# toverainc/willow-inference-server

Hardware: AMD Instinct MI355X
Metric: realtime_multiple (audio_ms / infer_ms), Whisper large-v2 beam=5, 3.84 s clip (higher is better)
Workload: dtype f16; 1 GPU; whisper-large beam=5 clip=3sec (3840 ms) batch=1/GPU, PCM resident in HBM -> ids on host; parallelism=1 independent replicas (utterance sharding, no data-path collective)

## Files before the change

### include/wis_hip.h

```cpp
#ifndef WIS_HIP_H
#define WIS_HIP_H

#include <stddef.h>
#include <stdint.h>

#ifdef __cplusplus
extern "C" {
#endif

#define WIS_ABI_VERSION 1

#define WIS_OK             0
#define WIS_E_ARG         -1
#define WIS_E_FORMAT      -2
#define WIS_E_NOMEM       -3
#define WIS_E_CHECKSUM    -4
#define WIS_E_HIP         -5
#define WIS_E_STATE       -6
#define WIS_E_UNSUPPORTED -7

#define WIS_SAMPLE_RATE 16000
#define WIS_N_FFT       400
#define WIS_HOP         160
#define WIS_N_MELS      80
// ... 136 lines not shown
int wis_align_last_timing(wis_model_t* m, float* ms);
int wis_op_dtw(int device, const float* x, int N, int M, int32_t* text_idx, int32_t* time_idx, int32_t* len);
int wis_op_align_matrix(int device, const float* q, const void* kx_f16, int T_tokens, int n_heads_sel, int T, int frames, int width, float* out);
int wis_debug_tree_logits(wis_model_t* m, const float* input, int input_kind, const int32_t* prompt, int P, int beam,
                          const int32_t* tok, const int32_t* org, int n_steps, float* logits);

int wis_debug_search(wis_model_t* m, const float* logits, int n_steps, int B, const wis_gen_opts_t* opts,
                     int32_t* out_ids, int32_t* out_len, float* out_score, int32_t* out_finish_step, int32_t* out_parent);
int wis_debug_search_n(wis_model_t* m, const float* logits, int n_steps, int B, const wis_gen_opts_t* opts, const uint64_t* seeds, const uint32_t* noise,
                       int32_t* out_ids, int32_t* out_len, float* out_score, int32_t* out_finish_step, int32_t* out_parent);

int wis_debug_handoff(wis_model_t* m, int raise_flag, int* retries, int* spin_disabled);
int wis_debug_graph_count(wis_model_t* m, int* count);
int wis_debug_sa_long(wis_model_t* m, int form);

typedef struct {
  float logmel_ms, encoder_ms, crosskv_ms, prefill_ms, decode_ms, total_ms;
  int32_t decode_steps;
  int32_t decode_steps_needed;
} wis_timing_t;
int wis_last_timing(const wis_model_t* m, wis_timing_t* t);

int wis_debug_phase_cycles(wis_model_t* m, int B, int beam, int pos, uint64_t* out);

int wis_debug_timeline(wis_model_t* m, int B, int beam, int pos, int use_graph, uint64_t* out, int n_out);
int wis_debug_sampling_cycles(wis_model_t* m, uint64_t* out);

int wis_bench_weight_stream(wis_model_t* m, int M, int passes, float* total_ms, int* launches_per_pass,
                            double* bytes_per_pass);

int wis_dev_alloc(int device, size_t bytes, void** out);
int wis_dev_free(int device, void* p);
int wis_dev_h2d(int device, void* dst, const void* src, size_t bytes);
int wis_dev_d2h(int device, void* dst, const void* src, size_t bytes);
int wis_dev_sync(int device);
int wis_dev_copy_peer(int dst_device, void* dst, int src_device, const void* src, size_t bytes);

int wis_op_gemm(int device, const void* A_f16, int lda, const void* W_f16, const float* bias,
                const float* residual, void* C, int M, int N, int K, int flags);
int wis_op_layernorm(int device, const float* x, const float* gamma, const float* beta,
                     void* y_f16, int M, int d);
int wis_op_enc_attention(int device, const void* qk_f16, const void* vt_f16, void* out_f16,
                         int B, int T, int Tpad, int H);
int wis_op_enc_attention_ex(int device, const void* qk_f16, const void* vt_f16, void* out_f16,
                            int B, int T, int Tpad, int H, int form);
int wis_op_gemv(int device, const void* x, const float* gamma, const float* beta,
// ... 91 lines not shown
```

### willow-inference-server_amd/csrc/dec_kernels.hip

```cpp
#include <string.h>
#include "common.hpp"
#include "kernels.hpp"

namespace wis {

__global__ void pack_gemv_kernel(const f16* __restrict__ W, f16* __restrict__ Wp, int N, int Npad, int K, int n_scale, float scale, int rows) {
  const int ksteps = K / 32;
  const size_t total = (size_t)Npad * ksteps * 4;
  for (size_t idx = (size_t)blockIdx.x * blockDim.x + threadIdx.x; idx < total; idx += (size_t)gridDim.x * blockDim.x) {
    const int row = (int)(idx % rows);
    size_t t = idx / rows;
    const int kq = (int)(t & 3); t >>= 2;
    const int ks = (int)(t % ksteps), nt = (int)(t / ksteps);
    const int n = rows * nt + row, k = 32 * ks + 8 * kq;
    f16x8 v;
    if (n < N) {
      v = *reinterpret_cast<const f16x8*>(W + (size_t)n * K + k);
      if (n < n_scale) {
#pragma unroll
        for (int j = 0; j < 8; ++j) v[j] = (f16)((float)v[j] * scale);
      }
    } else {
#pragma unroll
      for (int j = 0; j < 8; ++j) v[j] = (f16)0.f;
// ... 495 lines not shown
      if ((lane >> 4) == 0 && m < M && rows * tile < p.N) *reinterpret_cast<float2*>(p.stat_out + ((size_t)m * (p.N >> 4) + tile) * 2) = make_float2(t1, t2);
    }
  }
  stamp(pf, 6);
  if (tid == 0) tl_end(p.prof);
#undef WIS_ROW_OF
}
#define WIS_GV_LEAD(q) (q).x, (q).x2, (q).Wp, (q).M, (q).N, (q).K, (q).xsplit
#define WIS_GV_LEAD_DECL(s) const void* s##x, const void* s##x2, const f16* s##Wp, int s##M, int s##N, int s##K, int s##xsplit
#define WIS_GV_LEAD_APPLY(q, s) (q).x = s##x; (q).x2 = s##x2; (q).Wp = s##Wp; (q).M = s##M; (q).N = s##N; (q).K = s##K; (q).xsplit = s##xsplit
template <int MB, int MODE, int SC, int RM, bool W8, int NT = 1, int NC = 16>
__global__ __launch_bounds__(256) void gemv_kernel(WIS_GV_LEAD_DECL(l_), int KC, GemvP p) {
  extern __shared__ __attribute__((aligned(16))) char smem[];
  WIS_GV_LEAD_APPLY(p, l_);
  gemv_body<MB, MODE, SC, RM, W8, NT, NC>(p, KC, blockIdx.x, smem);
}
template <int SCA, int SCB>
__global__ __launch_bounds__(256) void gemv_dual_kernel(int nA, int M, const void* ax, const f16* aWp, const void* bx, const void* bx2, const f16* bWp, int bxsplit,
                                                        GemvP pa, GemvP pb) {
  extern __shared__ __attribute__((aligned(16))) char smem[];
  if ((int)blockIdx.x < nA) { pa.x = ax; pa.x2 = nullptr; pa.Wp = aWp; pa.M = M; pa.K = SCA * 128; gemv_body<1, 2, SCA, 1, false>(pa, SCA * 128, blockIdx.x, smem); }
  else { pb.x = bx; pb.x2 = bx2; pb.Wp = bWp; pb.M = M; pb.K = SCB * 128; pb.xsplit = bxsplit; gemv_body<1, 2, SCB, 1, false>(pb, SCB * 128, (int)blockIdx.x - nA, smem); }
}
int launch_gemv_dual(hipStream_t st, const GemvP& pa, const GemvP& pb) {
  if (pa.M != pb.M || pa.M < 1 || pa.M > 16 || pa.x2 || pa.wscale || pb.wscale || (pa.flags & (GV_LN | GV_QKV)) || (pb.flags & (GV_LN | GV_QKV))) { set_error("gemv_dual: unsupported pair"); return WIS_E_UNSUPPORTED; }
  if (pa.M * (pa.K / 8) > 13 * 256 || pb.M * (pb.K / 8) > 13 * 256 || pa.K % 128 || pb.K % 128) { set_error("gemv_dual: rows do not fit the register staging (M=%d K=%d/%d)", pa.M, pa.K, pb.K); return WIS_E_UNSUPPORTED; }
  const int sa = pa.K / 128, sb = pb.K / 128;
  const size_t aux = (size_t)4 * 64 * 16 + MAX_ROWS * 8 + 4 * 16 * 4 + 16;
  const int Kmax = pa.K > pb.K ? pa.K : pb.K;
  const size_t lds = (((size_t)pa.M * (Kmax + 8) * 2 + 15) & ~(size_t)15) + aux;
  if (lds > 65536) { set_error("gemv_dual: LDS"); return WIS_E_UNSUPPORTED; }
  const int nA = cdiv(pa.N, 16), nB = cdiv(pb.N, 16);
  dim3 grid(nA + nB), block(256);
  GemvP a = pa, b = pb; a.rows = 16; b.rows = 16;
  if (sa == 10 && sb == 20) hipLaunchKernelGGL((gemv_dual_kernel<10, 20>), grid, block, lds, st, nA, a.M, a.x, a.Wp, b.x, b.x2, b.Wp, b.xsplit, a, b);
  else if (sa == 8 && sb == 16) hipLaunchKernelGGL((gemv_dual_kernel<8, 16>), grid, block, lds, st, nA, a.M, a.x, a.Wp, b.x, b.x2, b.Wp, b.xsplit, a, b);
  else if (sa == 6 && sb == 12) hipLaunchKernelGGL((gemv_dual_kernel<6, 12>), grid, block, lds, st, nA, a.M, a.x, a.Wp, b.x, b.x2, b.Wp, b.xsplit, a, b);
  else if (sa == 4 && sb == 8) hipLaunchKernelGGL((gemv_dual_kernel<4, 8>), grid, block, lds, st, nA, a.M, a.x, a.Wp, b.x, b.x2, b.Wp, b.xsplit, a, b);
  else if (sa == 3 && sb == 6) hipLaunchKernelGGL((gemv_dual_kernel<3, 6>), grid, block, lds, st, nA, a.M, a.x, a.Wp, b.x, b.x2, b.Wp, b.xsplit, a, b);
  else { set_error("gemv_dual: K=%d/%d not instantiated", pa.K, pb.K); return WIS_E_UNSUPPORTED; }
  return WIS_OK;
}

#define GV_IN_ORDER() __builtin_amdgcn_sched_barrier(0x104)
template <int CTRL>
__device__ __forceinline__ f16x8 nc5_rot(const u32x4& w) {
  u32x4 r;
#pragma unroll
  for (int e = 0; e < 4; ++e) r[e] = (unsigned)__builtin_amdgcn_update_dpp(0, (int)w[e], CTRL, 0xf, 0xf, false);
  return *reinterpret_cast<const f16x8*>(&r);
}
__device__ __forceinline__ f32x4 ld4_f32(const float* p) { f32x4 v; __builtin_memcpy(&v, p, 16); return v; }
__device__ __forceinline__ f32x4 add4_f32(const f32x4& a, const f32x4& b) { return f32x4{a[0] + b[0], a[1] + b[1], a[2] + b[2], a[3] + b[3]}; }
__device__ __forceinline__ void st_nc5_f32(float* p, const f32x4& v, int kq) { if (kq) p[3] = v[3]; else __builtin_memcpy(p, &v, 16); }
__device__ __forceinline__ void st_nc5_f16(f16* p, const f32x4& v, int kq) {
  const f16x4 h = {(f16)v[0], (f16)v[1], (f16)v[2], (f16)v[3]};
  if (kq) p[3] = h[3]; else __builtin_memcpy(p, &h, 8);
}
// ... 50 lines not shown
    if (p.flags & GV_RESID) ep_res = ld4_f32(reinterpret_cast<const float*>(p.y) + o);
  }
  *reinterpret_cast<f32x4*>(red + ((size_t)wave * 64 + lane) * 4) = acc;
  __syncthreads();
  stamp(pf, 5);
  if (wave == 0) {
    f32x4 s = f32x4{0.f, 0.f, 0.f, 0.f};
#pragma unroll
    for (int w = 0; w < 4; ++w) s = add4_f32(s, *reinterpret_cast<const f32x4*>(red + ((size_t)w * 64 + lane) * 4));
    if (ep_ok) {
      if (kq) s[3] = s[0];
      s = add4_f32(s, ep_bias);
      if (p.flags & GV_GELU) { s[0] = gelu_erf(s[0]); s[1] = gelu_erf(s[1]); s[2] = gelu_erf(s[2]); s[3] = gelu_erf(s[3]); }
      if (p.flags & GV_RESID) {
        const f32x4 r = add4_f32(ep_res, s);
        st_nc5_f32(reinterpret_cast<float*>(p.y) + o, r, kq);
        if (p.y16) st_nc5_f16(p.y16 + o, r, kq);
      } else if (p.flags & GV_OUT_F32) st_nc5_f32(reinterpret_cast<float*>(p.y) + o, s, kq);
      else st_nc5_f16(reinterpret_cast<f16*>(p.y) + o, s, kq);
    }
  }
  stamp(pf, 6);
  if (tid == 0) tl_end(p.prof);
}
int launch_gemv(hipStream_t st, const GemvP& p) {
  if (p.M < 1 || p.M > 16 || p.K % 128 || (p.N % 4 && p.rows != 5)) { set_error("gemv: M=%d N=%d K=%d unsupported (the LDS-staged form holds one 16-row block; more rows take launch_gemv_frag)", p.M, p.N, p.K); return WIS_E_UNSUPPORTED; }
  int KC = p.K;
  const size_t aux = (size_t)4 * 64 * 16 + MAX_ROWS * 8 + 4 * 16 * 4 + 16;
  while ((size_t)p.M * (KC + 8) * 2 + aux > 65536) {
    int next = 0;
    for (int c = KC - 128; c >= 128; c -= 128) if (p.K % c == 0) { next = c; break; }
    if (!next) { set_error("gemv: cannot chunk K=%d for M=%d", p.K, p.M); return WIS_E_UNSUPPORTED; }
    KC = next;
  }
  const size_t lds = (((size_t)p.M * (KC + 8) * 2 + 15) & ~(size_t)15) + aux;
  const int rows = p.rows ? p.rows : 16;
  GemvP pp = p; pp.rows = rows;
  const int npad = cdiv(p.N, rows) * rows;
  dim3 grid(npad / rows), block(256);
  int mode = 0;
  if (p.flags & GV_LN) {
    if (p.M > 8 || p.K > 2048 || KC != p.K || !p.csum) { set_error("gemv: fused LayerNorm needs M <= 8, K <= 2048 and the folded column sums (M=%d K=%d)", p.M, p.K); return WIS_E_UNSUPPORTED; }
  }
  if (p.flags & GV_LN16) {
    if ((p.flags & GV_LN) || p.M > 8 || p.K > 2048 || p.K % 8 || KC != p.K || !p.csum) {
      set_error("gemv: the LayerNorm fold on f16 rows needs column sums, M <= 8, K <= 2048 (M=%d K=%d)", p.M, p.K); return WIS_E_UNSUPPORTED; }
// ... 2338 lines not shown
```

### willow-inference-server_amd/csrc/kernels.hpp

```cpp
#pragma once
#include "common.hpp"

namespace wis {

struct GemmP {
  const f16* A; int64_t a_bs; int a_rs; int a_rpb;
  const f16* W;
  int M, N, K;
  int klen;
  int n_span = 0, n_period = 0, n_phase = 0;
};
static inline GemmP gemm_plain(const f16* A, int lda, const f16* W, int M, int N, int K) {
  GemmP p; p.A = A; p.a_bs = 0; p.a_rs = lda; p.a_rpb = 0x7fffffff; p.W = W; p.M = M; p.N = N; p.K = K; p.klen = 0; return p;
}
int launch_layernorm(hipStream_t st, const float* x, const float* gamma, const float* beta, f16* y, int M, int d);
int launch_gemm_generic(hipStream_t st, const GemmP& p, const float* bias, const float* resid, void* C, int flags);
int launch_gemm_splitk_resid(hipStream_t st, const GemmP& p, int splits, float* scratch, const float* bias, const float* resid, float* X,
                             const float* ln_gamma = nullptr, const float* ln_beta = nullptr, f16* Y = nullptr);
int launch_gemm_conv1(hipStream_t st, const GemmP& p, const float* bias, f16* C, int T);
int launch_gemm_conv2(hipStream_t st, const GemmP& p, const float* bias, const float* pos, float* X, int T);
int launch_gemm_qkv(hipStream_t st, const GemmP& p, const float* bias, f16* qk, f16* vt, int d, int T, int Tpad, int H);
int launch_gemm_crosskv(hipStream_t st, const GemmP& p, const float* bias, f16* kx, f16* vt, int d, int T, int Tpad, int H, int64_t kx_lstride, int64_t vt_lstride);
int launch_enc_attention(hipStream_t st, const f16* qk, const f16* vt, f16* out, int B, int T, int Tpad, int H, float* part = nullptr, unsigned* counters = nullptr,
                         size_t part_cap = 0);
// ... 21 lines not shown
  const void* x;
  const float* gamma; const float* beta;
  const float* csum;
  const f16* Wp; const float* bias;
  const float* wscale;
  void* y;
  int M, N, K, flags;
  float* q; f16* kc; f16* vc; const int* slot; const int* pos; int d; int ctx;
  unsigned long long* prof;
  int rows;
  const void* x2; int xsplit;
  f16* y16;
  int xmb;
  const float* stat_in;
  float* stat_out;
  f16* y_xf;
  int ymb;
  int ksplit; float* kpart; unsigned* kcnt;
  int mb0, mbi;
  int wks, wk0;
};
int launch_gemv(hipStream_t st, const GemvP& p);
int launch_gemv_dual(hipStream_t st, const GemvP& pa, const GemvP& pb);
int launch_gemv_frag(hipStream_t st, const GemvP& p);
int launch_gemv_frag3(hipStream_t st, const GemvP* p, int n);
__host__ __device__ static inline size_t xf_index(int m, int k, int MB) {
  return ((size_t)((k >> 5) * MB + (m >> 4)) * 64 + (m & 15) + 16 * ((k >> 3) & 3)) * 8 + (k & 7);
}
constexpr size_t xf_elems(int K, int MB) { return (size_t)(K / 32) * MB * 64 * 8; }
int launch_xf_pack(hipStream_t st, const void* x, int x_f16, f16* xf, float* stat, int M, int K, int MB);
int launch_dec_embed_xf(hipStream_t st, const f16* emb, const f16* pos_emb, const int* tok, const int* pos, float* x, f16* xf, float* stat, int M, int d, int MB);
int launch_fold_ln(hipStream_t st, f16* W, const float* gamma, const float* beta, float* bias, float* csum, int N, int K, int n_scale, float qscale);
int launch_csum8(hipStream_t st, const f16* W, const float* scale, float* csum, int N, int K, int n_scale, float qscale);
int launch_pack_gemv8(hipStream_t st, const f16* W, unsigned char* Wp, float* scale, int N, int Npad, int K, int n_scale, float qscale);
int launch_pack_gemv(hipStream_t st, const f16* W, f16* Wp, int N, int Npad, int K, int n_scale, float scale, int rows = 16);
int launch_pack_gemv_nc8(hipStream_t st, const f16* W, f16* Wp, int N, int Npad, int K);
bool gemv_nc8_shape(int M, int N, int K);
size_t gemv_nc5_elems(int N, int K, int kw);
int launch_pack_gemv_nc5(hipStream_t st, const f16* W, f16* Wp, int N, int K, int kw);
bool gemv_nc5_shape(int M, int N, int K, int flags);
int gemv_rows_for(int N, int K);

int launch_dec_embed(hipStream_t st, const f16* emb, const f16* pos_emb, const int* tok, const int* pos, float* x, int M, int d, f16* xh = nullptr);
struct SelfAttnP {
  const float* q = nullptr; const f16* kc = nullptr; const f16* vc = nullptr; const int* pos = nullptr; f16* out = nullptr;
  int M = 0, H = 0, d = 0, ctx = 0, rpu = 0, sstride = 0, rmul = 0;
// ... 93 lines not shown
```

### willow-inference-server_amd/csrc/model.hip

```cpp
#include <math.h>
#include <stdlib.h>
#include <string.h>
#include <algorithm>
#include <atomic>
#include <mutex>
#include <memory>
#include <string>
#include <vector>

#include "common.hpp"
#include "kernels.hpp"
#include "model.hpp"

using namespace wis;

namespace wis {

__global__ void convert_kernel(const void* __restrict__ src, int src_f16, void* __restrict__ dst, int dst_f16,
                               int64_t rows, int64_t cols, int64_t dst_ld, int64_t n_scale, float scale) {
  const int64_t total = rows * cols;
  for (int64_t i = (int64_t)blockIdx.x * blockDim.x + threadIdx.x; i < total; i += (int64_t)gridDim.x * blockDim.x) {
    const int64_t r = i / cols, c = i - r * cols;
    float v = src_f16 ? (float)reinterpret_cast<const f16*>(src)[i] : reinterpret_cast<const float*>(src)[i];
    if (r < n_scale) v *= scale;
// ... 286 lines not shown
    if (hipMemsetAsync(b_proj, 0, ((size_t)V + 64) * 4, m->st) != hipSuccess) { set_error("memset failed"); rc = WIS_E_HIP; break; }
    if ((rc = to_packed(m, L, "decoder/embeddings/weight", V, d, tmp, 0, 1.f, m->dec_ln_g, m->dec_ln_b, b_proj, &m->proj, &m->n_vocab_pad))) break;
    m->proj.N = m->n_vocab_pad;
    m->dec.resize(c.n_dec_layers);
    if ((rc = dalloc(m, &m->w_ckv_all, (size_t)c.n_dec_layers * 2 * d * d))) break;
    if ((rc = dalloc(m, &m->b_ckv_all, (size_t)c.n_dec_layers * 2 * d))) break;
    for (int l = 0; l < c.n_dec_layers && !rc; ++l) {
      const std::string p = "decoder/layer_" + std::to_string(l) + "/";
      DecLayerW& w = m->dec[l];
      if ((rc = to_f32(m, L, p + "self_attention/layer_norm/gamma", d, &w.ln1_g))) break;
      if ((rc = to_f32(m, L, p + "self_attention/layer_norm/beta", d, &w.ln1_b))) break;
      if ((rc = load_proj(m, L, p + "self_attention/linear_0", 3 * d, d, tmp, d, qs, w.ln1_g, w.ln1_b, &w.qkv))) break;
      if ((rc = load_proj(m, L, p + "self_attention/linear_1", d, d, tmp, 0, 1.f, nullptr, nullptr, &w.out))) break;
      if ((rc = to_f32(m, L, p + "attention/layer_norm/gamma", d, &w.ln2_g))) break;
      if ((rc = to_f32(m, L, p + "attention/layer_norm/beta", d, &w.ln2_b))) break;
      if ((rc = load_proj(m, L, p + "attention/linear_0", d, d, tmp, d, qs, w.ln2_g, w.ln2_b, &w.cq))) break;
      if (m->cq_fold) {
        TensorSrc so; if ((rc = L.get(p + "self_attention/linear_1/weight", d, d, &so))) break;
        f16* p_cqo = nullptr; float* b_cqo = nullptr;
        if ((rc = dalloc(m, &p_cqo, (size_t)d * 2 * d))) break;
        if ((rc = dalloc(m, &b_cqo, (size_t)d))) break;
        if ((rc = build_cq_fold(m->st, tmp, so.p, so.f16, w.out.bias, d, qs, fcat, fwot, fwqo, p_cqo, b_cqo))) break;
        w.cqo = DecProj{p_cqo, nullptr, b_cqo, nullptr, d, 2 * d, 16};
      }
      w.w_ckv = m->w_ckv_all + (size_t)l * 2 * d * d; w.b_ckv = m->b_ckv_all + (size_t)l * 2 * d;
      if ((rc = to_f16_mat(m, L, p + "attention/linear_1/weight", 2 * d, d, &w.w_ckv))) break;
      if ((rc = to_f32(m, L, p + "attention/linear_1/bias", 2 * d, &w.b_ckv))) break;
      if ((rc = load_proj(m, L, p + "attention/linear_2", d, d, tmp, 0, 1.f, nullptr, nullptr, &w.cout))) break;
      if ((rc = add_nc8_image(m, tmp, &w.cout))) break;
      if ((rc = to_f32(m, L, p + "ffn/layer_norm/gamma", d, &w.ln3_g))) break;
      if ((rc = to_f32(m, L, p + "ffn/layer_norm/beta", d, &w.ln3_b))) break;
      bool nc5 = false;
      if ((rc = load_proj(m, L, p + "ffn/linear_0", 4 * d, d, tmp, 0, 1.f, w.ln3_g, w.ln3_b, &w.f1))) break;
      if ((rc = load_proj(m, L, p + "ffn/linear_1", d, 4 * d, tmp, 0, 1.f, nullptr, nullptr, &w.f2))) break;
      if ((rc = add_nc5_image(m, tmp, &w.f2, &nc5))) break;
      if (!nc5 && (rc = add_nc8_image(m, tmp, &w.f2))) break;
    }
  } while (0);
  hipError_t e = hipStreamSynchronize(m->st);
  hipFree(tmp); hipFree(fcat); hipFree(fwot); hipFree(fwqo);
  if (rc) return rc;
  if (e != hipSuccess) { set_error("weight conversion failed: %s", hipGetErrorString(e)); return WIS_E_HIP; }
  return WIS_OK;
}

static int frag_ksplit_setting() {
// ... 257 lines not shown
  }
  return WIS_OK;
}


GemvP gemv_small(const DecProj& p, const void* x, void* y, int M, int flags) {
  GemvP g; memset(&g, 0, sizeof(g));
  g.x = x; g.csum = p.csum; g.Wp = p.Wp; g.wscale = p.scale; g.bias = p.bias; g.y = y; g.M = M; g.N = p.N; g.K = p.K; g.flags = flags; g.rows = p.rows;
  if (p.Wp8 && !(flags & ~(GV_RESID | GV_OUT_F32 | GV_GELU)) && gemv_nc8_shape(M, p.N, p.K)) { g.Wp = p.Wp8; g.rows = 8; }
  if (p.Wp5 && !p.scale && !p.csum && gemv_nc5_shape(M, p.N, p.K, flags)) { g.Wp = p.Wp5; g.rows = 5; }
  return g;
}
GemvP gemv_frag(const DecProj& p, const void* xf, int M, int flags) {
  GemvP g; memset(&g, 0, sizeof(g));
  g.x = xf; g.csum = p.csum; g.Wp = p.Wp; g.wscale = p.scale; g.bias = p.bias; g.M = M; g.N = p.N; g.K = p.K; g.flags = flags; g.xmb = cdiv(M, 16); g.rows = 16;
  return g;
}
void out_cq_dual(const DecLayerW& w, const f16* a, const f16* xh, float* x1, float* stat, float* q, int M, GemvP* ga, GemvP* gb) {
  const int d = w.out.K;
  memset(ga, 0, sizeof(*ga));
  ga->x = a; ga->Wp = w.out.Wp; ga->bias = w.out.bias; ga->y = x1; ga->M = M; ga->N = d; ga->K = d; ga->flags = GV_RESID; ga->stat_out = stat;
  memset(gb, 0, sizeof(*gb));
  gb->x = xh; gb->x2 = a; gb->xsplit = d; gb->Wp = w.cqo.Wp; gb->bias = w.cqo.bias; gb->y = q; gb->M = M; gb->N = d; gb->K = w.cqo.K; gb->flags = GV_OUT_F32;
}
void out_cq_frag3(const DecLayerW& w, const f16* af, const f16* xf, float* x1, float* stat, float* q, float* q2, int M, GemvP g3[3]) {
  const int d = w.out.K;
  g3[0] = gemv_frag(w.out, af, M, GV_RESID);
  g3[0].wscale = nullptr; g3[0].y = x1; g3[0].ymb = g3[0].xmb; g3[0].stat_out = stat;
  g3[1] = gemv_frag(w.cqo, xf, M, GV_OUT_F32);
  g3[1].K = d; g3[1].y = q; g3[1].wks = w.cqo.K / 32; g3[1].wk0 = 0;
  g3[2] = gemv_frag(w.cqo, af, M, GV_OUT_F32);
  g3[2].K = d; g3[2].bias = nullptr; g3[2].y = q2; g3[2].wks = w.cqo.K / 32; g3[2].wk0 = d / 32;
}

GemvP frag_resid(const DecProj& p, const f16* xf, float* y, f16* y_xf, float* stat_out, int M) {
  GemvP g = gemv_frag(p, xf, M, GV_RESID);
  g.y = y; g.y_xf = y_xf; g.ymb = g.xmb; g.stat_out = stat_out;
  return g;
}
GemvP frag_ln_f32(const DecProj& p, const f16* xf, const float* stat_in, float* y, int M) {
  GemvP g = gemv_frag(p, xf, M, GV_LN | GV_OUT_F32);
  g.stat_in = stat_in; g.y = y;
  return g;
}
GemvP frag_ln_gelu_xf(const DecProj& p, const f16* xf, const float* stat_in, f16* y_xf, int M) {
  GemvP g = gemv_frag(p, xf, M, GV_LN | GV_GELU);
// ... 90 lines not shown
  const int ln = ln16 ? GV_LN16 : GV_LN;
  auto ln_x = [&](const f16* x16) { return ln16 ? (const void*)x16 : (const void*)m->dx; };
  WIS_RET(launch_dec_embed(st, m->emb, m->dec_pos, m->rm.tok, m->rm.pos, m->dx, M, d, fold ? m->dxh : nullptr));
  SelfAttnP sa;
  sa.q = m->dq; sa.pos = m->rm.pos; sa.out = m->dao; sa.M = M; sa.H = H; sa.d = d; sa.ctx = ctx; sa.rpu = R; sa.sstride = sstride; sa.rmul = rmul; sa.nb = m->sa_nb;
  sa_shared_prefix(m, &sa);
  CrossAttnP ca;
  ca.q = m->dq; ca.out = m->dao; ca.part = m->part; ca.counters = m->counters; ca.B = B; ca.R = R; ca.H = H; ca.d = d; ca.T = T; ca.Tpad = m->Tpad; ca.chunks = chunks;
  ca.gran = m->spin_now ? m->ca_gran : nullptr; ca.epoch = m->ca_epoch;
  for (int l = 0; l < c.n_dec_layers; ++l) {
    const DecLayerW& w = m->dec[l];
    unsigned long long* pr = (m->prof_on && (l == 0 || m->prof_all)) ? m->d_prof + (size_t)l * 8 * 16 : nullptr;
    GemvP g = gemv_small(w.qkv, ln_x(m->dxh), nullptr, M, ln | GV_QKV);
    g.q = m->dq; g.kc = m->kc[l]; g.vc = m->vc[l]; g.slot = m->rm.slot; g.pos = m->rm.pos; g.d = d; g.ctx = ctx;
    g.prof = pr;
    WIS_RET(launch_gemv(st, g));
    sa.kc = m->kc[l]; sa.vc = m->vc[l]; sa.prof = pr ? pr + 16 : nullptr;
    WIS_RET(launch_dec_self_attn(st, sa));
    ca.kx = m->kx[l]; ca.vt = m->vx[l]; ca.prof = pr ? pr + 64 : nullptr;
    if (fold) {
      GemvP ga, gb;
      out_cq_dual(w, m->dao, m->dxh, m->dx, m->dstat, m->dq, M, &ga, &gb);
      ga.prof = pr ? pr + 32 : nullptr;
      WIS_RET(launch_gemv_dual(st, ga, gb));
      CrossAttnP cf = ca;
      cf.xres = m->dstat; cf.qcs = w.cq.csum; cf.qb = w.cq.bias; cf.xres_is_stat = 1;
      WIS_RET(launch_dec_cross_attn(st, cf));
    } else {
    g = gemv_small(w.out, m->dao, m->dx, M, GV_RESID);
    g.prof = pr ? pr + 32 : nullptr;
    WIS_RET(launch_gemv(st, g));
    g = gemv_small(w.cq, m->dx, m->dq, M, GV_LN | GV_OUT_F32);
    g.prof = pr ? pr + 48 : nullptr;
    WIS_RET(launch_gemv(st, g));
    WIS_RET(launch_dec_cross_attn(st, ca));
    }
    g = gemv_small(w.cout, m->dao, m->dx, M, GV_RESID);
    g.prof = pr ? pr + 80 : nullptr;
    if (ln16) g.y16 = m->dln;
    WIS_RET(launch_gemv(st, g));
    g = gemv_small(w.f1, ln_x(m->dln), m->dh, M, ln | GV_GELU);
    g.prof = pr ? pr + 96 : nullptr;
    WIS_RET(launch_gemv(st, g));
    g = gemv_small(w.f2, m->dh, m->dx, M, GV_RESID);
    g.prof = pr ? pr + 112 : nullptr;
    g.y16 = fold ? m->dxh : nullptr;
// ... 297 lines not shown
```

### willow-inference-server_amd/csrc/taps.hip

```cpp
#include <string.h>
#include <algorithm>
#include <vector>

#include "common.hpp"
#include "kernels.hpp"
#include "model.hpp"
#include "tap.hpp"

using namespace wis;

extern "C" {

int wis_debug_encode(wis_model_t* m, const float* input, int input_kind, int B, float* enc_out) {
  if (!m || !input || !enc_out) { set_error("wis_debug_encode: bad argument"); return WIS_E_ARG; }
  WIS_ENTER(m, "wis_debug_encode")
  WIS_HIP_CHECK(hipSetDevice(m->device));
  WIS_RET(check_batch(m, B, 1));
  WIS_RET(stage_input(m, input, input_kind, B));
  WIS_RET(run_encoder(m, B));
  const int64_t n = (int64_t)B * m->cfg.n_audio_ctx * m->cfg.d_model;
  launch_f16_to_f32(m->st, m->mem, m->x, n);
  WIS_HIP_CHECK(hipMemcpyAsync(enc_out, m->x, (size_t)n * 4, hipMemcpyDeviceToHost, m->st));
  WIS_HIP_CHECK(hipStreamSynchronize(m->st));
  return WIS_OK;
// ... 37 lines not shown
  if (!m || !out) { set_error("wis_debug_phase_cycles: bad argument"); return WIS_E_ARG; }
  if (!WIS_TAPS) { set_error("tuning taps are not compiled in (rebuild with WIS_EXTRA_HIPFLAGS=-DWIS_TAPS=1)"); return WIS_E_UNSUPPORTED; }
  WIS_ENTER(m, "wis_debug_phase_cycles")
  WIS_HIP_CHECK(hipSetDevice(m->device));
  WIS_RET(check_batch(m, B, beam));
  SpinClaim claim(m, B);
  const int Mrows = B * beam, ctx = m->cfg.n_text_ctx;
  if (pos < 0 || pos >= ctx) { set_error("bad pos"); return WIS_E_ARG; }
  WIS_HIP_CHECK(hipStreamSynchronize(m->st));
  WIS_RET(single_row_setup(m, Mrows, std::vector<int>(Mrows, 100), pos));
  WIS_HIP_CHECK(hipMemsetAsync(m->d_prof, 0, 8 * 16 * 8, m->st));
  WIS_RET(dec_forward(m, Mrows, beam, B, false, beam, 1));
  m->prof_on = true;
  int rc = dec_forward(m, Mrows, beam, B, false, beam, 1);
  m->prof_on = false;
  WIS_RET(rc);
  static const int rows_small[6] = {0, 2, 4, 1, 6, 7}, rows_frag[6] = {0, 2, 4, 5, 6, 7};
  const int* rows = Mrows > 8 ? rows_frag : rows_small;
  for (int i = 0; i < 6; ++i)
    WIS_HIP_CHECK(hipMemcpyAsync(out + i * 16, m->d_prof + rows[i] * 16, 16 * 8, hipMemcpyDeviceToHost, m->st));
  bool gave_up = false;
  WIS_RET(spin_gave_up(m, &gave_up));
  if (gave_up) { set_error("wis_debug_phase_cycles: the granule hand-off gave up during the tap; stamps are not valid"); return WIS_E_STATE; }
  return WIS_OK;
}

int wis_debug_sampling_cycles(wis_model_t* m, uint64_t* out) {
  if (!m || !out) { set_error("wis_debug_sampling_cycles: bad argument"); return WIS_E_ARG; }
  if (!WIS_TAPS) { set_error("tuning taps are not compiled in (rebuild with WIS_EXTRA_HIPFLAGS=-DWIS_TAPS=1)"); return WIS_E_UNSUPPORTED; }
  WIS_HIP_CHECK(hipSetDevice(m->device));
  WIS_HIP_CHECK(hipMemcpy(out, m->d_prof + (size_t)m->cfg.n_dec_layers * 8 * 16, 2 * 16 * 8, hipMemcpyDeviceToHost));
  return WIS_OK;
}

int wis_debug_timeline(wis_model_t* m, int B, int beam, int pos, int use_graph, uint64_t* out, int n_out) {
  if (!m || !out) { set_error("wis_debug_timeline: bad argument"); return WIS_E_ARG; }
  if (!WIS_TAPS) { set_error("tuning taps are not compiled in (rebuild with WIS_EXTRA_HIPFLAGS=-DWIS_TAPS=1)"); return WIS_E_UNSUPPORTED; }
  WIS_ENTER(m, "wis_debug_timeline")
  WIS_HIP_CHECK(hipSetDevice(m->device));
  WIS_RET(check_batch(m, B, beam));
  SpinClaim claim(m, B);
  const int Mrows = B * beam, ctx = m->cfg.n_text_ctx, nk = m->cfg.n_dec_layers * 8;
  if (pos < 0 || pos >= ctx || n_out < nk) { set_error("wis_debug_timeline: bad pos / out size (need %d rows)", nk); return WIS_E_ARG; }
  WIS_HIP_CHECK(hipStreamSynchronize(m->st));
  WIS_RET(single_row_setup(m, Mrows, std::vector<int>(Mrows, 100), pos));
  std::vector<unsigned long long> init((size_t)nk * 16, 0ull);
// ... 368 lines not shown
int wis_op_gemv_out_cq(int device, const void* a, const float* x0, const void* Wo, const float* bo, const void* Wq, const float* bq, const float* gamma, const float* beta,
                       float* x1, float* stat, float* q, float* q2, float* qcs, float* qb, int M, int d, int force_frag) {
  Tap t(device, "wis_op_gemv_out_cq"); WIS_RET(t.rc);
  const bool frag = M > 8 || force_frag;
  if (!a || !x0 || !Wo || !bo || !Wq || !bq || !gamma || !beta || !x1 || !stat || !q || !qcs || !qb || (frag && !q2) || M < 1 || M > MAX_ROWS || d < 128 || d % 128) {
    set_error("wis_op_gemv_out_cq: bad argument"); return WIS_E_ARG; }
  hipStream_t st = t.st;
  const int MB = cdiv(M, 16);
  const float qs = 0.125f;
  f16 *wtmp = nullptr, *fcat = nullptr, *fwot = nullptr, *fwqo = nullptr, *p_cqo = nullptr, *p_out = nullptr, *xh = nullptr, *xf = nullptr, *af = nullptr; float* b_cqo = nullptr;
  WIS_RET(t.get(&wtmp, (size_t)d * d)); WIS_RET(t.get(&fcat, (size_t)2 * d * d)); WIS_RET(t.get(&fwot, (size_t)d * d)); WIS_RET(t.get(&fwqo, (size_t)d * d));
  WIS_RET(t.get(&p_cqo, (size_t)2 * d * d)); WIS_RET(t.get(&p_out, (size_t)d * d)); WIS_RET(t.get(&b_cqo, (size_t)d));
  if (frag) { WIS_RET(t.get(&xf, xf_elems(d, MB), true)); WIS_RET(t.get(&af, xf_elems(d, MB), true)); }
  else WIS_RET(t.get(&xh, (size_t)M * d));
  hipMemcpyAsync(wtmp, Wq, (size_t)d * d * 2, hipMemcpyDeviceToDevice, st);
  launch_convert(st, bq, 0, qb, 0, d, 1, 1, d, qs);
  hipMemsetAsync(qcs, 0, (size_t)d * 4, st);
  DecLayerW w{};
  w.out = DecProj{p_out, nullptr, bo, nullptr, d, d, gemv_rows_for(d, d)};
  w.cqo = DecProj{p_cqo, nullptr, b_cqo, nullptr, d, 2 * d, 16};
  WIS_RET(prep_projection(st, wtmp, d, d, d, d, qs, gamma, beta, qb, qcs, nullptr, nullptr, 16));
  WIS_RET(launch_pack_gemv(st, reinterpret_cast<const f16*>(Wo), p_out, d, d, d, 0, 1.f, w.out.rows));
  WIS_RET(build_cq_fold(st, wtmp, Wo, 1, bo, d, qs, fcat, fwot, fwqo, p_cqo, b_cqo));
  hipMemcpyAsync(x1, x0, (size_t)M * d * 4, hipMemcpyDeviceToDevice, st);
  if (!frag) {
    launch_convert(st, x0, 0, xh, 1, M, d, d, 0, 1.f);
    GemvP ga, gb;
    out_cq_dual(w, reinterpret_cast<const f16*>(a), xh, x1, stat, q, M, &ga, &gb);
    return t.finish(launch_gemv_dual(st, ga, gb));
  }
  WIS_RET(launch_xf_pack(st, x0, 0, xf, nullptr, M, d, MB));
  WIS_RET(launch_xf_pack(st, a, 1, af, nullptr, M, d, MB));
  GemvP g3[3];
  out_cq_frag3(w, af, xf, x1, stat, q, q2, M, g3);
  return t.finish(launch_gemv_frag3(st, g3, 3));
}

int wis_op_mel_to_image(int device, const float* mel, void* img_f16, int B, int n_mels) {
  Tap t(device, "wis_op_mel_to_image"); WIS_RET(t.rc);
  if (!mel || !img_f16 || B < 1) { set_error("wis_op_mel_to_image: bad argument"); return WIS_E_ARG; }
  return t.finish(launch_mel_to_image(t.st, mel, reinterpret_cast<f16*>(img_f16), B, n_mels));
}
int wis_op_enc_conv(int device, int which, const void* img_f16, const void* W, int w_is_f16, const float* bias, const float* pos, void* out,
                    int B, int T, int Cin, int N) {
  Tap t(device, "wis_op_enc_conv"); WIS_RET(t.rc);
  if (!img_f16 || !W || !bias || !out || B < 1 || T < 1 || N < 128 || (which != 1 && which != 2) || (which == 2 && !pos) || (int64_t)B * (2 * (int64_t)T + 2) > 0x7fffffff) {
// ... 122 lines not shown
```

### willow-inference-server_amd/wis_hip/_lib.py

```python
import ctypes as C
import os

import numpy as np

_HERE = os.path.dirname(os.path.abspath(__file__))
LIB_PATH = os.environ.get("WIS_LIB_PATH") or os.path.join(os.path.dirname(_HERE), "lib", "libwis_hip.so")

WIS_OK = 0
WIS_IN_MEL_HOST, WIS_IN_MEL_DEV, WIS_IN_PCM_HOST, WIS_IN_PCM_DEV = 0, 1, 2, 3
WIS_IN_ENC_DEV, WIS_IN_ENC_HOST = 4, 5
WIS_DT_F32, WIS_DT_F16 = 0, 1
N_SAMPLES, N_FRAMES, N_MELS = 480000, 3000, 80


class WisError(RuntimeError):
    def __init__(self, code, msg):
        super().__init__(f"libwis_hip error {code}: {msg}")
        self.code = code


class Config(C.Structure):
    _fields_ = [(n, C.c_int32) for n in ("d_model", "n_heads", "n_enc_layers", "n_dec_layers", "n_vocab", "n_audio_ctx",
                                          "n_text_ctx", "n_mels", "max_batch", "max_beam", "eot", "sot", "no_timestamps",
                                          "no_speech")] + [
# ... 78 lines not shown
    ("wis_detect_language", _i, [_vp, _vp, _i, _i, _fp]),
    ("wis_encode", _i, [_vp, _vp, _i, _i, _vp, _fp]),
    ("wis_debug_encode", _i, [_vp, _vp, _i, _i, _fp]),
    ("wis_debug_logits", _i, [_vp, _vp, _i, _i, C.POINTER(C.c_int32), _i, _fp]),
    ("wis_debug_logits_rows", _i, [_vp, _vp, _i, _i, C.POINTER(C.c_int32), _i, _i, _fp]),
    ("wis_model_set_alignment_heads", _i, [_vp, C.POINTER(C.c_int32), _i]),
    ("wis_align", _i, [_vp, _vp, _i, _i, C.POINTER(C.c_int32), _i, C.POINTER(C.c_int32), C.POINTER(C.c_int32), C.POINTER(C.c_int32), _i,
                       C.POINTER(C.c_int32), C.POINTER(C.c_int32), C.POINTER(C.c_int32), _fp]),
    ("wis_debug_align_matrix", _i, [_vp, _vp, _i, _i, C.POINTER(C.c_int32), _i, C.POINTER(C.c_int32), C.POINTER(C.c_int32), C.POINTER(C.c_int32), _i, _fp]),
    ("wis_align_last_timing", _i, [_vp, _fp]),
    ("wis_op_dtw", _i, [_i, _vp, _i, _i, _vp, _vp, _vp]),
    ("wis_op_align_matrix", _i, [_i, _vp, _vp, _i, _i, _i, _i, _i, _vp]),
    ("wis_debug_tree_logits", _i, [_vp, _vp, _i, C.POINTER(C.c_int32), _i, _i, C.POINTER(C.c_int32), C.POINTER(C.c_int32), _i, _fp]),
    ("wis_debug_search", _i, [_vp, _vp, _i, _i, C.POINTER(GenOpts), C.POINTER(C.c_int32), C.POINTER(C.c_int32), _fp, C.POINTER(C.c_int32), C.POINTER(C.c_int32)]),
    ("wis_debug_search_n", _i, [_vp, _vp, _i, _i, C.POINTER(GenOpts), C.POINTER(C.c_uint64), C.POINTER(C.c_uint32), C.POINTER(C.c_int32), C.POINTER(C.c_int32), _fp,
                                C.POINTER(C.c_int32), C.POINTER(C.c_int32)]),
    ("wis_debug_handoff", _i, [_vp, _i, C.POINTER(_i), C.POINTER(_i)]),
    ("wis_debug_graph_count", _i, [_vp, C.POINTER(_i)]),
    ("wis_debug_sa_long", _i, [_vp, _i]),
    ("wis_last_timing", _i, [_vp, C.POINTER(Timing)]),
    ("wis_debug_phase_cycles", _i, [_vp, _i, _i, _i, C.POINTER(C.c_uint64)]),
    ("wis_debug_timeline", _i, [_vp, _i, _i, _i, _i, C.POINTER(C.c_uint64), _i]),
    ("wis_debug_sampling_cycles", _i, [_vp, C.POINTER(C.c_uint64)]),
    ("wis_bench_weight_stream", _i, [_vp, _i, _i, _fp, C.POINTER(_i), C.POINTER(C.c_double)]),
    ("wis_dev_alloc", _i, [_i, _sz, C.POINTER(_vp)]),
    ("wis_dev_free", _i, [_i, _vp]),
    ("wis_dev_h2d", _i, [_i, _vp, _vp, _sz]),
    ("wis_dev_d2h", _i, [_i, _vp, _vp, _sz]),
    ("wis_dev_sync", _i, [_i]),
    ("wis_dev_copy_peer", _i, [_i, _vp, _i, _vp, _sz]),
    ("wis_op_gemm", _i, [_i, _vp, _i, _vp, _vp, _vp, _vp, _i, _i, _i, _i]),
    ("wis_op_layernorm", _i, [_i, _vp, _vp, _vp, _vp, _i, _i]),
    ("wis_op_enc_attention", _i, [_i, _vp, _vp, _vp, _i, _i, _i, _i]),
    ("wis_op_enc_attention_ex", _i, [_i, _vp, _vp, _vp, _i, _i, _i, _i, _i]),
    ("wis_op_gemv", _i, [_i, _vp, _vp, _vp, _vp, _vp, _vp, _i, _i, _i, _i]),
    ("wis_op_gemv_cols", _i, [_i, _vp, _vp, _vp, _vp, _vp, _i, _i, _i, _i, _i]),
    ("wis_op_dec_self_attn", _i, [_i, _vp, _vp, _vp, _vp, _vp, _i, _i, _i, _i, _i, _i]),
    ("wis_op_dec_cross_attn", _i, [_i, _vp, _vp, _vp, _vp, _i, _i, _i, _i, _i]),
    ("wis_op_dec_cross_attn_folded", _i, [_i, _vp, _vp, _vp, _vp, _vp, _vp, _vp, _i, _i, _i, _i, _i]),
    ("wis_op_dec_cross_attn_stat", _i, [_i] + [_vp] * 8 + [_i] * 8),
    ("wis_op_dec_self_attn_ex", _i, [_i, _vp, _vp, _vp, _vp, _vp, _i, _i, _i, _i, _i, _i, _i, _i, _vp, _i, _i, _vp]),
    ("wis_op_gemv_qkv", _i, [_i] + [_vp] * 10 + [_i] * 3),
    ("wis_op_gemv_out_cq", _i, [_i] + [_vp] * 14 + [_i] * 3),
    ("wis_op_gemv_frag_stage", _i, [_i, _i, _vp, _i, _i] + [_vp] * 5 + [_i] + [_vp] * 3 + [_i] * 4),
    ("wis_op_dec_embed", _i, [_i, _vp, _vp, C.POINTER(C.c_int32), C.POINTER(C.c_int32), _vp, _vp, _vp, _vp, _i, _i, _i, _i]),
    ("wis_op_mel_to_image", _i, [_i, _vp, _vp, _i, _i]),
# ... 99 lines not shown
```

Before: 152.9 x realtime.

## Add dedicated out-proj + cross-Q dual GEMV kernel with eight-column tiles

Adds a specialised kernel for the fused decoder out-projection plus folded cross-attention Q projection. It stages activations through registers and spreads each arm's K across the four waves with an LDS reduction. For large's width (d=1280, M<=8) it also packs a second copy of the cross-Q weights into eight-column tiles, using DPP lane rotation so the B arm launches twice as many blocks and fills more CUs. This costs extra weight memory and a new code path, and adds a profiling tap for the new arm.

Result: faster. 155.6 x realtime, median of 6 (+1.8%).

```diff
diff --git a/include/wis_hip.h b/include/wis_hip.h
--- a/include/wis_hip.h
+++ b/include/wis_hip.h
@@ -182,6 +182,7 @@
 int wis_last_timing(const wis_model_t* m, wis_timing_t* t);
 
 int wis_debug_phase_cycles(wis_model_t* m, int B, int beam, int pos, uint64_t* out);
+int wis_debug_phase_cycles_cq_arm(wis_model_t* m, uint64_t* out);
 
 int wis_debug_timeline(wis_model_t* m, int B, int beam, int pos, int use_graph, uint64_t* out, int n_out);
 int wis_debug_sampling_cycles(wis_model_t* m, uint64_t* out);
diff --git a/willow-inference-server_amd/csrc/dec_kernels.hip b/willow-inference-server_amd/csrc/dec_kernels.hip
--- a/willow-inference-server_amd/csrc/dec_kernels.hip
+++ b/willow-inference-server_amd/csrc/dec_kernels.hip
@@ -541,6 +541,8 @@
   if ((int)blockIdx.x < nA) { pa.x = ax; pa.x2 = nullptr; pa.Wp = aWp; pa.M = M; pa.K = SCA * 128; gemv_body<1, 2, SCA, 1, false>(pa, SCA * 128, blockIdx.x, smem); }
   else { pb.x = bx; pb.x2 = bx2; pb.Wp = bWp; pb.M = M; pb.K = SCB * 128; pb.xsplit = bxsplit; gemv_body<1, 2, SCB, 1, false>(pb, SCB * 128, (int)blockIdx.x - nA, smem); }
 }
+static bool out_cq_shape(const GemvP& pa, const GemvP& pb);
+static void launch_out_cq(hipStream_t st, dim3 grid, dim3 block, size_t lds, int nA, const GemvP& a, const GemvP& b);
 int launch_gemv_dual(hipStream_t st, const GemvP& pa, const GemvP& pb) {
   if (pa.M != pb.M || pa.M < 1 || pa.M > 16 || pa.x2 || pa.wscale || pb.wscale || (pa.flags & (GV_LN | GV_QKV)) || (pb.flags & (GV_LN | GV_QKV))) { set_error("gemv_dual: unsupported pair"); return WIS_E_UNSUPPORTED; }
   if (pa.M * (pa.K / 8) > 13 * 256 || pb.M * (pb.K / 8) > 13 * 256 || pa.K % 128 || pb.K % 128) { set_error("gemv_dual: rows do not fit the register staging (M=%d K=%d/%d)", pa.M, pa.K, pb.K); return WIS_E_UNSUPPORTED; }
@@ -549,10 +551,13 @@
   const int Kmax = pa.K > pb.K ? pa.K : pb.K;
   const size_t lds = (((size_t)pa.M * (Kmax + 8) * 2 + 15) & ~(size_t)15) + aux;
   if (lds > 65536) { set_error("gemv_dual: LDS"); return WIS_E_UNSUPPORTED; }
-  const int nA = cdiv(pa.N, 16), nB = cdiv(pb.N, 16);
+  const bool b8 = pb.rows == 8;
+  if (b8 && !(out_cq_shape(pa, pb) && out_cq_nc8_shape(pa.M, pa.K))) { set_error("gemv_dual: the eight-column image serves the out-projection + cross-Q pair of large's width, <= 8 rows (M=%d K=%d/%d)", pa.M, pa.K, pb.K); return WIS_E_UNSUPPORTED; }
+  const int nA = cdiv(pa.N, 16), nB = b8 ? pb.N / 8 : cdiv(pb.N, 16);
   dim3 grid(nA + nB), block(256);
-  GemvP a = pa, b = pb; a.rows = 16; b.rows = 16;
-  if (sa == 10 && sb == 20) hipLaunchKernelGGL((gemv_dual_kernel<10, 20>), grid, block, lds, st, nA, a.M, a.x, a.Wp, b.x, b.x2, b.Wp, b.xsplit, a, b);
+  GemvP a = pa, b = pb; a.rows = 16; b.rows = b8 ? 8 : 16;
+  if (out_cq_shape(pa, pb)) launch_out_cq(st, grid, block, lds, nA, a, b);
+  else if (sa == 10 && sb == 20) hipLaunchKernelGGL((gemv_dual_kernel<10, 20>), grid, block, lds, st, nA, a.M, a.x, a.Wp, b.x, b.x2, b.Wp, b.xsplit, a, b);
   else if (sa == 8 && sb == 16) hipLaunchKernelGGL((gemv_dual_kernel<8, 16>), grid, block, lds, st, nA, a.M, a.x, a.Wp, b.x, b.x2, b.Wp, b.xsplit, a, b);
   else if (sa == 6 && sb == 12) hipLaunchKernelGGL((gemv_dual_kernel<6, 12>), grid, block, lds, st, nA, a.M, a.x, a.Wp, b.x, b.x2, b.Wp, b.xsplit, a, b);
   else if (sa == 4 && sb == 8) hipLaunchKernelGGL((gemv_dual_kernel<4, 8>), grid, block, lds, st, nA, a.M, a.x, a.Wp, b.x, b.x2, b.Wp, b.xsplit, a, b);
@@ -649,6 +654,126 @@
   }
   stamp(pf, 6);
   if (tid == 0) tl_end(p.prof);
+}
+
+template <int SC, bool ARM_B, int NC = 16>
+__device__ __forceinline__ void out_cq_arm(const GemvP& p, const int nt, char* smem) {
+  static_assert(NC == 16 || (NC == 8 && ARM_B), "eight-column tiles: arm B");
+  constexpr int SW = ARM_B ? 2 * SC : SC, K = SW * 128, xstr = K + 8, c8 = K / 8, s8 = c8 / 2;
+  constexpr int RQ = NC == 8 ? SW / 2 : SW;
+  constexpr int NXH = (8 * c8 + 255) / 256;
+  const int M = p.M;
+  f16* xs = reinterpret_cast<f16*>(smem);
+  float* red = reinterpret_cast<float*>(smem + (((size_t)M * xstr * 2 + 15) & ~(size_t)15));
+  const int tid = threadIdx.x, lane = tid & 63, wave = tid >> 6;
+  unsigned long long* pf = (nt == 0 && tid == 0) ? p.prof : nullptr;
+  if (tid == 0) tl_begin(p.prof);
+  stamp(pf, 0);
+  const int nx = M * c8;
+  const u32x4* x8 = reinterpret_cast<const u32x4*>(p.x);
+  const u32x4* y8 = reinterpret_cast<const u32x4*>(p.x2);
+  u32x4 xh[NXH];
+#pragma unroll
+  for (int i = 0; i < NXH; ++i) {
+    const int idx = min(tid + 256 * i, nx - 1);
+    if (ARM_B) {
+      const int row = idx / c8, col = idx - row * c8;
+      const u32x4* src = col < s8 ? x8 + (row * s8 + col) : y8 + (row * s8 + (col - s8));
+      xh[i] = *src;
+    } else xh[i] = x8[idx];
+  }
+  GV_IN_ORDER();
+  const u32x4* wq = reinterpret_cast<const u32x4*>(p.Wp) + ((size_t)nt * 4 + wave) * RQ * 64 + lane;
+  u32x4 wf[RQ];
+#pragma unroll
+  for (int u = 0; u < RQ; ++u) { wf[u] = __builtin_nontemporal_load(wq + (size_t)u * 64); GV_IN_ORDER(); }
+  stamp(pf, 1);
+#pragma unroll
+  for (int i = 0; i < NXH; ++i) {
+    const int idx = tid + 256 * i;
+    if (idx < nx) { const int row = idx / c8, k8 = idx - row * c8; *reinterpret_cast<u32x4*>(xs + (size_t)row * xstr + k8 * 8) = xh[i]; }
+  }
+  __syncthreads();
+  stamp(pf, 3);
+  f32x4 acc = f32x4{0.f, 0.f, 0.f, 0.f};
+  const f16* xw = xs + ((lane & 15) < M ? (lane & 15) : M - 1) * xstr + 8 * (lane >> 4) + wave * SW * 32;
+  if (ARM_B) {
+    f16x8 xb[SW];
+#pragma unroll
+    for (int k = 0; k < SW; ++k) xb[k] = *reinterpret_cast<const f16x8*>(xw + k * 32);
+    __builtin_amdgcn_sched_barrier(0);
+#pragma unroll
+    for (int u = 0; u < RQ; ++u) {
+      if (NC == 8) {
+        acc = __builtin_amdgcn_mfma_f32_16x16x32_f16(*reinterpret_cast<const f16x8*>(&wf[u]), xb[2 * u], acc, 0, 0, 0);
+        acc = __builtin_amdgcn_mfma_f32_16x16x32_f16(nc5_rot<0x128>(wf[u]), xb[NC == 8 ? 2 * u + 1 : 0], acc, 0, 0, 0);
+      } else acc = __builtin_amdgcn_mfma_f32_16x16x32_f16(*reinterpret_cast<const f16x8*>(&wf[u]), xb[u], acc, 0, 0, 0);
+      GV_IN_ORDER();
+    }
+  } else {
+#pragma unroll
+    for (int u = 0; u < SW; ++u)
+      acc = __builtin_amdgcn_mfma_f32_16x16x32_f16(*reinterpret_cast<const f16x8*>(&wf[u]), *reinterpret_cast<const f16x8*>(xw + u * 32), acc, 0, 0, 0);
+  }
+  stamp(pf, 4);
+  const int ep_m = lane & 15, ep_n = NC * nt + 4 * (lane >> 4);
+  const bool ep_ok = tid < 64 && ep_m < M && ep_n < p.N && 4 * (lane >> 4) < NC;
+  float4 ep_bias = make_float4(0.f, 0.f, 0.f, 0.f), ep_res = ep_bias;
+  if (ep_ok) {
+    if (p.bias) ep_bias = *reinterpret_cast<const float4*>(p.bias + ep_n);
+    if (!ARM_B) ep_res = *reinterpret_cast<const float4*>(reinterpret_cast<const float*>(p.y) + (size_t)ep_m * p.N + ep_n);
+  }
+  *reinterpret_cast<float4*>(red + ((size_t)wave * 64 + lane) * 4) = make_float4(acc[0], acc[1], acc[2], acc[3]);
+  __syncthreads();
+  stamp(pf, 5);
+  if (tid < 64) {
+    float4 s = make_float4(0.f, 0.f, 0.f, 0.f);
+#pragma unroll
+    for (int w = 0; w < 4; ++w) {
+      const float4 t = *reinterpret_cast<const float4*>(red + ((size_t)w * 64 + lane) * 4);
+      s.x += t.x; s.y += t.y; s.z += t.z; s.w += t.w;
+    }
+    float4 rsum = make_float4(0.f, 0.f, 0.f, 0.f);
+    if (ep_ok) {
+      s.x += ep_bias.x; s.y += ep_bias.y; s.z += ep_bias.z; s.w += ep_bias.w;
+      const size_t o = (size_t)ep_m * p.N + ep_n;
+      if (ARM_B) {
+        *reinterpret_cast<float4*>(reinterpret_cast<float*>(p.y) + o) = s;
+      } else {
+        const float4 r = make_float4(ep_res.x + s.x, ep_res.y + s.y, ep_res.z + s.z, ep_res.w + s.w);
+        rsum = r;
+        *reinterpret_cast<float4*>(reinterpret_cast<float*>(p.y) + o) = r;
+      }
+    }
+    if (!ARM_B && p.stat_out) {
+      float t1 = ep_ok ? (rsum.x + rsum.y) + (rsum.z + rsum.w) : 0.f;
+      t1 += __shfl_xor(t1, 16); t1 += __shfl_xor(t1, 32);
+      float t2 = 0.f;
+      if (ep_ok) { const float ml = t1 * 0.0625f, a_ = rsum.x - ml, b_ = rsum.y - ml, c_ = rsum.z - ml, e_ = rsum.w - ml; t2 = (a_ * a_ + b_ * b_) + (c_ * c_ + e_ * e_); }
+      t2 += __shfl_xor(t2, 16); t2 += __shfl_xor(t2, 32);
+      if ((lane >> 4) == 0 && ep_m < M && 16 * nt < p.N) *reinterpret_cast<float2*>(p.stat_out + ((size_t)ep_m * (p.N >> 4) + nt) * 2) = make_float2(t1, t2);
+    }
+  }
+  stamp(pf, 6);
+  if (tid == 0) tl_end(p.prof);
+}
+template <int SC, int NCB>
+__global__ __launch_bounds__(256) void gemv_out_cq_kernel(int nA, int M, const void* ax, const f16* aWp, const void* bx, const void* bx2, const f16* bWp, int bxsplit,
+                                                          GemvP pa, GemvP pb) {
+  extern __shared__ __attribute__((aligned(16))) char smem[];
+  (void)bxsplit;
+  if ((int)blockIdx.x < nA) { pa.x = ax; pa.x2 = nullptr; pa.Wp = aWp; pa.M = M; out_cq_arm<SC, false>(pa, blockIdx.x, smem); }
+  else { pb.x = bx; pb.x2 = bx2; pb.Wp = bWp; pb.M = M; out_cq_arm<SC, true, NCB>(pb, (int)blockIdx.x - nA, smem); }
+}
+bool out_cq_nc8_shape(int M, int d) { return d == 1280 && M >= 1 && M <= 8 && d / 16 + d / 8 <= device_cu_count(); }
+static bool out_cq_shape(const GemvP& pa, const GemvP& pb) {
+  return pa.M <= 8 && pa.flags == GV_RESID && pb.flags == GV_OUT_F32 && pb.K == 2 * pa.K && pb.x2 && pb.xsplit == pa.K && !pa.y16 && !pb.y16 && !pb.stat_out &&
+         pa.N % 16 == 0 && pb.N % 16 == 0 && (pa.K == 1280 || pa.K == 384);
+}
+static void launch_out_cq(hipStream_t st, dim3 grid, dim3 block, size_t lds, int nA, const GemvP& a, const GemvP& b) {
+  if (b.rows == 8) hipLaunchKernelGGL((gemv_out_cq_kernel<10, 8>), grid, block, lds, st, nA, a.M, a.x, a.Wp, b.x, b.x2, b.Wp, b.xsplit, a, b);
+  else if (a.K == 1280) hipLaunchKernelGGL((gemv_out_cq_kernel<10, 16>), grid, block, lds, st, nA, a.M, a.x, a.Wp, b.x, b.x2, b.Wp, b.xsplit, a, b);
+  else hipLaunchKernelGGL((gemv_out_cq_kernel<3, 16>), grid, block, lds, st, nA, a.M, a.x, a.Wp, b.x, b.x2, b.Wp, b.xsplit, a, b);
 }
 int launch_gemv(hipStream_t st, const GemvP& p) {
   if (p.M < 1 || p.M > 16 || p.K % 128 || (p.N % 4 && p.rows != 5)) { set_error("gemv: M=%d N=%d K=%d unsupported (the LDS-staged form holds one 16-row block; more rows take launch_gemv_frag)", p.M, p.N, p.K); return WIS_E_UNSUPPORTED; }
diff --git a/willow-inference-server_amd/csrc/kernels.hpp b/willow-inference-server_amd/csrc/kernels.hpp
--- a/willow-inference-server_amd/csrc/kernels.hpp
+++ b/willow-inference-server_amd/csrc/kernels.hpp
@@ -67,6 +67,7 @@
 };
 int launch_gemv(hipStream_t st, const GemvP& p);
 int launch_gemv_dual(hipStream_t st, const GemvP& pa, const GemvP& pb);
+bool out_cq_nc8_shape(int M, int d);
 int launch_gemv_frag(hipStream_t st, const GemvP& p);
 int launch_gemv_frag3(hipStream_t st, const GemvP* p, int n);
 __host__ __device__ static inline size_t xf_index(int m, int k, int MB) {
diff --git a/willow-inference-server_amd/csrc/model.hip b/willow-inference-server_amd/csrc/model.hip
--- a/willow-inference-server_amd/csrc/model.hip
+++ b/willow-inference-server_amd/csrc/model.hip
@@ -332,6 +332,12 @@
         if ((rc = dalloc(m, &b_cqo, (size_t)d))) break;
         if ((rc = build_cq_fold(m->st, tmp, so.p, so.f16, w.out.bias, d, qs, fcat, fwot, fwqo, p_cqo, b_cqo))) break;
         w.cqo = DecProj{p_cqo, nullptr, b_cqo, nullptr, d, 2 * d, 16};
+        if (!m->w8 && out_cq_nc8_shape(1, d)) {
+          f16* p8 = nullptr;
+          if ((rc = dalloc(m, &p8, (size_t)d * 2 * d))) break;
+          if ((rc = launch_pack_gemv_nc8(m->st, fcat, p8, d, d, 2 * d))) break;
+          w.cqo.Wp8 = p8;
+        }
       }
       w.w_ckv = m->w_ckv_all + (size_t)l * 2 * d * d; w.b_ckv = m->b_ckv_all + (size_t)l * 2 * d;
       if ((rc = to_f16_mat(m, L, p + "attention/linear_1/weight", 2 * d, d, &w.w_ckv))) break;
@@ -635,6 +641,7 @@
   ga->x = a; ga->Wp = w.out.Wp; ga->bias = w.out.bias; ga->y = x1; ga->M = M; ga->N = d; ga->K = d; ga->flags = GV_RESID; ga->stat_out = stat;
   memset(gb, 0, sizeof(*gb));
   gb->x = xh; gb->x2 = a; gb->xsplit = d; gb->Wp = w.cqo.Wp; gb->bias = w.cqo.bias; gb->y = q; gb->M = M; gb->N = d; gb->K = w.cqo.K; gb->flags = GV_OUT_F32;
+  if (w.cqo.Wp8 && out_cq_nc8_shape(M, d)) { gb->Wp = w.cqo.Wp8; gb->rows = 8; }
 }
 void out_cq_frag3(const DecLayerW& w, const f16* af, const f16* xf, float* x1, float* stat, float* q, float* q2, int M, GemvP g3[3]) {
   const int d = w.out.K;
@@ -771,6 +778,7 @@
       GemvP ga, gb;
       out_cq_dual(w, m->dao, m->dxh, m->dx, m->dstat, m->dq, M, &ga, &gb);
       ga.prof = pr ? pr + 32 : nullptr;
+      gb.prof = pr ? pr + 48 : nullptr;
       WIS_RET(launch_gemv_dual(st, ga, gb));
       CrossAttnP cf = ca;
       cf.xres = m->dstat; cf.qcs = w.cq.csum; cf.qb = w.cq.bias; cf.xres_is_stat = 1;
diff --git a/willow-inference-server_amd/csrc/taps.hip b/willow-inference-server_amd/csrc/taps.hip
--- a/willow-inference-server_amd/csrc/taps.hip
+++ b/willow-inference-server_amd/csrc/taps.hip
@@ -83,6 +83,14 @@
   bool gave_up = false;
   WIS_RET(spin_gave_up(m, &gave_up));
   if (gave_up) { set_error("wis_debug_phase_cycles: the granule hand-off gave up during the tap; stamps are not valid"); return WIS_E_STATE; }
+  return WIS_OK;
+}
+
+int wis_debug_phase_cycles_cq_arm(wis_model_t* m, uint64_t* out) {
+  if (!m || !out) { set_error("wis_debug_phase_cycles_cq_arm: bad argument"); return WIS_E_ARG; }
+  if (!WIS_TAPS) { set_error("tuning taps are not compiled in (rebuild with WIS_EXTRA_HIPFLAGS=-DWIS_TAPS=1)"); return WIS_E_UNSUPPORTED; }
+  WIS_HIP_CHECK(hipSetDevice(m->device));
+  WIS_HIP_CHECK(hipMemcpy(out, m->d_prof + 3 * 16, 16 * 8, hipMemcpyDeviceToHost));
   return WIS_OK;
 }
 
@@ -497,6 +505,12 @@
   WIS_RET(prep_projection(st, wtmp, d, d, d, d, qs, gamma, beta, qb, qcs, nullptr, nullptr, 16));
   WIS_RET(launch_pack_gemv(st, reinterpret_cast<const f16*>(Wo), p_out, d, d, d, 0, 1.f, w.out.rows));
   WIS_RET(build_cq_fold(st, wtmp, Wo, 1, bo, d, qs, fcat, fwot, fwqo, p_cqo, b_cqo));
+  if (out_cq_nc8_shape(1, d)) {
+    f16* p8 = nullptr;
+    WIS_RET(t.get(&p8, (size_t)2 * d * d));
+    WIS_RET(launch_pack_gemv_nc8(st, fcat, p8, d, d, 2 * d));
+    w.cqo.Wp8 = p8;
+  }
   hipMemcpyAsync(x1, x0, (size_t)M * d * 4, hipMemcpyDeviceToDevice, st);
   if (!frag) {
     launch_convert(st, x0, 0, xh, 1, M, d, d, 0, 1.f);
diff --git a/willow-inference-server_amd/wis_hip/_lib.py b/willow-inference-server_amd/wis_hip/_lib.py
--- a/willow-inference-server_amd/wis_hip/_lib.py
+++ b/willow-inference-server_amd/wis_hip/_lib.py
@@ -124,6 +124,7 @@
     ("wis_debug_phase_cycles", _i, [_vp, _i, _i, _i, C.POINTER(C.c_uint64)]),
     ("wis_debug_timeline", _i, [_vp, _i, _i, _i, _i, C.POINTER(C.c_uint64), _i]),
     ("wis_debug_sampling_cycles", _i, [_vp, C.POINTER(C.c_uint64)]),
+    ("wis_debug_phase_cycles_cq_arm", _i, [_vp, C.POINTER(C.c_uint64)]),
     ("wis_bench_weight_stream", _i, [_vp, _i, _i, _fp, C.POINTER(_i), C.POINTER(C.c_double)]),
     ("wis_dev_alloc", _i, [_i, _sz, C.POINTER(_vp)]),
     ("wis_dev_free", _i, [_i, _vp]),
```
